# XiaoJiang-Phy/TensorCrossInterpolation.jl

Hardware: AMD Instinct MI355X
Metric: rrLU GFLOP/s at (m,n,r)=(8192,8192,256) (higher is better)
Workload: dtype f64

## Files before the change

### tensorcrossinterpolation.jl_amd/csrc/tci_rrlu.hip

```cpp
#include <hip/hip_runtime.h>
#include <math.h>
#include <stdint.h>

#include <type_traits>

#include "tci_internal.h"
#include "tci_smalllu.h"

#ifndef TCI_PASS2_U
#define TCI_PASS2_U 4
#endif
#ifndef TCI_SH_HALF
#define TCI_SH_HALF 1
#endif
#ifndef TCI_PASS_SH_U
#define TCI_PASS_SH_U 2
#endif
#ifndef TCI_SH_MFMA
#define TCI_SH_MFMA TCI_SH_HALF
#endif
#ifndef TCI_SH_NT
#define TCI_SH_NT 0
#endif
#ifndef TCI_SH_TIGHT
// ... 816 lines not shown
    const int G = kP2StageCols / cb;
    constexpr int RL = kShRL, RH = RL / 2;
    typedef float fvec __attribute__((ext_vector_type(RL)));
    typedef shT svec __attribute__((ext_vector_type(RL)));
    const int r0 = tr * kRowsPerTile + slice * kShSliceRows + RL * lane;
    const int rb = r0 < m ? r0 : 0;
    const shT* const sbase = reinterpret_cast<const shT*>(g.S) + rb;
    const int cbs = __builtin_ctz(cb);
    auto chunk_col = [&](int g0, int h) -> int {
        const int it = g0 + ((h * U) >> cbs);
        return ((q + (rev ? ntc - 1 - it : it) * nq) << cbs) + ((h * U) & (cb - 1));
    };
    auto load_chunk = [&](int g0, int h, svec (&v)[U]) {
        const int j = chunk_col(g0, h);
#pragma unroll
        for (int u = 0; u < U; ++u)
            v[u] = *reinterpret_cast<const svec*>(sbase + (int64_t)min(j + u, n - 1) * lds);
    };
    auto stage_col = [&](int g0) -> int {
        const int gn = min(G, ntc - g0);
        const int lc = threadIdx.x;
        if (lc >= gn * cb) return -1;
        const int it = g0 + (lc >> cbs);
        return ((q + (rev ? ntc - 1 - it : it) * nq) << cbs) + (lc & (cb - 1));
    };
    int rp[RL];
#pragma unroll
    for (int t = 0; t < RL; ++t) rp[t] = r0 + t < m ? sel.rowpos[r0 + t] : -1;
    const int lrow = slice * kShSliceRows + RL * lane;
    int jst = ntc > 0 ? stage_col(0) : -1;
    int cpst = (jst >= 0 && jst < n) ? colpos[jst] : -1;
    svec va[U], vb[U];
    const int nch0 = ntc > 0 ? min(G, ntc) * cb / U : 0;
    if (rep < nch0) load_chunk(0, rep, va);
    if (rep + kShReps < nch0) load_chunk(0, rep + kShReps, vb);
    if (st->done) return false;
    const int a = (int)st->p, b = (int)st->q;
    const double piv = st->pval;
    const double ypr0 = g.A[a + (int64_t)((jst >= 0 && jst < n) ? jst : 0) * lda];
    unsigned inm = 0;
#pragma unroll
    for (int t = 0; t < RL; ++t) inm |= (rp[t] > k ? 1u : 0u) << t;
    const bool active = inm != 0;
    typedef float f2v __attribute__((ext_vector_type(2)));
    f2v xf[P][RH];
    {
        double xk[RL];
#pragma unroll
        for (int hh = 0; hh < RH; ++hh) {
            const double2 c0 = *reinterpret_cast<const double2*>(g.A + rb + 2 * hh + (int64_t)b * lda);
            xk[2 * hh] = c0.x;
            xk[2 * hh + 1] = c0.y;
        }
#pragma unroll
        for (int s = 0; s < P - 1; ++s) {
            double xs[RL];
#pragma unroll
            for (int hh = 0; hh < RH; ++hh) {
                const double2 u0 = *reinterpret_cast<const double2*>(g.X + (int64_t)s * ldx + rb + 2 * hh);
                xs[2 * hh] = u0.x;
                xs[2 * hh + 1] = u0.y;
                xf[s][hh] = f2v{(float)u0.x, (float)u0.y};
            }
            const double yv = g.Y[(int64_t)s * ldy + b];
#pragma unroll
            for (int t = 0; t < RL; ++t) xk[t] = __dsub_rn(xk[t], __dmul_rn(xs[t], yv));
        }
#pragma unroll
        for (int t = 0; t < RL; ++t)
            if (g.leftorth) xk[t] = xk[t] / piv;
#pragma unroll
        for (int hh = 0; hh < RH; ++hh) xf[P - 1][hh] = f2v{(float)xk[2 * hh], (float)xk[2 * hh + 1]};
        if (rep == 0) {
#pragma unroll
            for (int t = 0; t < RL; ++t) L.xk[lrow + t] = xk[t];
            if (q == 0) {
#pragma unroll
                for (int t = 0; t < RL; ++t)
                    if (inm >> t & 1) {
                        g.X[(int64_t)(P - 1) * ldx + r0 + t] = xk[t];
                        g.Lp[r0 + t + (int64_t)k * g.ldl] = xk[t];
                    }
            }
        }
    }
    PPROF(1);
    const bool wact = __any(active);
    const float margin = 0x1p-20f;
    float tau = 0.0f;
    auto approx = [&](int h, const svec (&v)[U]) -> float {
        float cm[RL];
#pragma unroll
        for (int t = 0; t < RL; ++t) cm[t] = 0.0f;
#pragma unroll
        for (int u = 0; u < U; ++u) {
            const int lc = h * U + u;
            if (L.cpos[lc] <= k) continue;
            const fvec vf = __builtin_convertvector(v[u], fvec);
            f2v w[RH];
#pragma unroll
            for (int hh = 0; hh < RH; ++hh) w[hh] = f2v{vf[2 * hh], vf[2 * hh + 1]};
#pragma unroll
            for (int s = 0; s < P; ++s) {
                const float y = L.yf[lc * P + s];
                const f2v yy = {y, y};
#pragma unroll
                for (int hh = 0; hh < RH; ++hh) w[hh] = __builtin_elementwise_fma(-xf[s][hh], yy, w[hh]);
            }
#pragma unroll
            for (int hh = 0; hh < RH; ++hh) {
                cm[2 * hh] = fmaxf(cm[2 * hh], fabsf(w[hh].x));
                cm[2 * hh + 1] = fmaxf(cm[2 * hh + 1], fabsf(w[hh].y));
            }
        }
        float c = 0.0f;
#pragma unroll
        for (int t = 0; t < RL; ++t)
            if (inm >> t & 1) c = fmaxf(c, cm[t]);
        return c;
    };
    auto examine = [&](int g0, int e0, int e1) {
#pragma unroll 1
        for (int z = 0; z < 2; ++z) {
            const int h = z ? e1 : e0;
            if (h < 0) continue;
            int rbx = rb;
            asm volatile("" : "+v"(rbx));
            const int j0 = chunk_col(g0, h);
#pragma unroll 1
            for (int u = 0; u < U; ++u) {
                const int lc = h * U + u;
                const int cp = L.cpos[lc];
                if (cp <= k) continue;
                const int j = j0 + u;
                const double* pa = g.A + rbx + (int64_t)j * lda;
                double v[RL];
#pragma unroll
                for (int hh = 0; hh < RH; ++hh) {
                    const double2 p0 = *reinterpret_cast<const double2*>(pa + 2 * hh);
                    v[2 * hh] = p0.x;
                    v[2 * hh + 1] = p0.y;
                }
#pragma unroll 1
                for (int s = 0; s < P - 1; ++s) {
                    const double y = L.ys[lc * P + s];
#pragma unroll
                    for (int hh = 0; hh < RH; ++hh) {
                        const double2 u0 = *reinterpret_cast<const double2*>(g.X + (int64_t)s * ldx + rbx + 2 * hh);
                        v[2 * hh] = __dsub_rn(v[2 * hh], __dmul_rn(u0.x, y));
                        v[2 * hh + 1] = __dsub_rn(v[2 * hh + 1], __dmul_rn(u0.y, y));
                    }
                }
                const double yk = L.ys[lc * P + P - 1];
#pragma unroll 1
                for (int t = 0; t < RL; ++t) {
                    if (!(inm >> t & 1)) continue;
                    const double vt = __dsub_rn(v[t], __dmul_rn(L.xk[lrow + t], yk));
                    const double a2 = __dmul_rn(vt, vt);
                    if (a2 >= best.v) cand_take(best, CandR{a2, vt, cp, sel.rowpos[r0 + t], j, r0 + t});
                }
            }
        }
    };
    auto test = [&](float c) -> bool {
        const float lb = fmaxf(c - eps, 0.0f);
        const float ts = __uint_as_float(__hip_atomic_load(&L.tau, __ATOMIC_RELAXED, __HIP_MEMORY_SCOPE_WORKGROUP));
        tau = fmaxf(tau, ts);
        if (lb > tau) {
            tau = lb;
            atomicMax(&L.tau, __float_as_uint(lb));
        }
        return c + eps >= tau - tau * margin;
    };
    for (int g0 = 0; g0 < ntc; g0 += G) {
        const int gn = min(G, ntc - g0);
        const int nch = gn * cb / U;
        if (g0 > 0) {
            jst = stage_col(g0);
            cpst = (jst >= 0 && jst < n) ? colpos[jst] : -1;
            if (wact) {
                if (rep < nch) load_chunk(g0, rep, va);
                if (rep + kShReps < nch) load_chunk(g0, rep + kShReps, vb);
            }
            __syncthreads();
        }
        if (jst >= 0) {
            int lc = threadIdx.x;
            asm volatile("" : "+v"(lc));
            L.cpos[lc] = cpst;
            if (cpst > k) {
                double yk = g0 == 0 ? ypr0 : g.A[a + (int64_t)jst * lda];
#pragma unroll
                for (int s = 0; s < P - 1; ++s) {
                    const double ysv = g.Y[(int64_t)s * ldy + jst];
                    L.ys[lc * P + s] = ysv;
                    L.yf[lc * P + s] = (float)(ysv * shs);
                    yk = __dsub_rn(yk, __dmul_rn(g.X[(int64_t)s * ldx + a], ysv));
                }
                if (!g.leftorth) yk = yk / piv;
                L.ys[lc * P + P - 1] = yk;
                L.yf[lc * P + P - 1] = (float)(yk * shs);
                if (tr == 0) {
                    g.Y[(int64_t)(P - 1) * ldy + jst] = yk;
                    g.Up[k + (int64_t)jst * g.ldu] = yk;
                }
            }
        }
        if (threadIdx.x < kShSlices) L.cnt[threadIdx.x] = 2 * kShReps;
        if (g0 == 0 && threadIdx.x == 0) L.tau = 0u;
        __syncthreads();
        if (g0 == 0) PPROF(2);
        auto grab = [&]() -> int {
            int h = 0;
            if (lane == 0) h = atomicAdd(&L.cnt[slice], 1);
            return __shfl(h, 0);
        };
        int h0 = rep, h1 = rep + kShReps;
        int ex0 = -1, ex1 = -1;
        if (g0 == 0) {
            float c0 = -1.0f, c1 = -1.0f;
            const int e0 = h0, e1 = h1;
            if (wact) {
                if (h0 < nch) {
                    c0 = approx(h0, va);
                    h0 = grab();
                    if (h0 < nch) load_chunk(g0, h0, va);
                }
                if (h1 < nch) {
                    c1 = approx(h1, vb);
                    h1 = grab();
                    if (h1 < nch) load_chunk(g0, h1, vb);
                }
                float lb = fmaxf(fmaxf(c0, c1) - eps, 0.0f);
#pragma unroll
                for (int off = 32; off >= 1; off >>= 1) lb = fmaxf(lb, __shfl_xor(lb, off));
                if (lane == 0) atomicMax(&L.tau, __float_as_uint(lb));
            }
            __syncthreads();
            if (!wact) continue;
            tau = __uint_as_float(L.tau);
            if (c0 >= 0.0f && c0 + eps >= tau - tau * margin) ex0 = e0;
            if (c1 >= 0.0f && c1 + eps >= tau - tau * margin) ex1 = e1;
        } else if (!wact) {
            continue;
        }
        for (;;) {
            if (ex0 >= 0 || ex1 >= 0) examine(g0, ex0, ex1);
            ex0 = ex1 = -1;
            if (h0 >= nch) break;
            {
                const float c = approx(h0, va);
                const int e = h0;
                h0 = grab();
                if (h0 < nch) load_chunk(g0, h0, va);
                if (test(c)) ex0 = e;
            }
            if (h1 < nch) {
                const float c = approx(h1, vb);
                const int e = h1;
                h1 = grab();
                if (h1 < nch) load_chunk(g0, h1, vb);
                if (test(c)) ex1 = e;
            }
        }
    }
    return true;
}

template <int P>
__global__ __launch_bounds__(kP2Threads) void k_pass_sh(PassK g, SelArgs sel) {
    __shared__ P2Lds<P> L;
    [[maybe_unused]] unsigned long long pt[8] = {0, 0, 0, 0, 0, 0, 0, 0};
    PPROF(0);
    const double* pv = sel.pivvals;
    const int t0 = g.k - P + 1;
    const double Mf = fabs(pv[t0]);
    double sumM = 0.0;
#pragma unroll
    for (int s = 0; s < P; ++s) sumM += fabs(pv[t0 + s]);
    const double mag = Mf + 2.0 * sumM;
    const double shs = sh_scale(sh_bound(pv, t0));
    double epsd = (double)(P + 3) * 0x1p-23 * mag * shs + (double)(P + 2) * 0x1p-124;
    if (kShHalf) epsd += 0x1p-11 * (1.0 + 0x1p-10) * Mf * shs + 0x1p-25;
    const bool shok = shs > 0.0 && mag < 0x1p100 &&
                      epsd < ldexp(fabs(pv[g.k]) * shs, -(kShHalf ? TCI_SH_TIGHT : 10));
    CandR best = cand_none();
    bool go;
    if (shok)
        go = pass_sh_body<P>(g, sel, L, best, (float)(epsd * (1.0 + 0x1p-20)), shs, pt);
    else
        go = pass2_body<P, false, false>(g, sel, L, best, pt);
    if (!go) return;
    PPROF(3);
    pass_tail<kP2Threads>(best, sel, g.cand, pt, g.m, P, 0);
}

constexpr int kMfRows = 64;
constexpr int kMfBlk = kMfRows / 16;
constexpr int kMfSlices = kRowsPerTile / kMfRows;
constexpr int kMfReps = kP2Threads / 64 / kMfSlices;
static_assert(kMfBlk == 4, "a lane's 16 loaded rows are 4 blocks of 4");

constexpr int kMfMaxP = 15;
constexpr int kMfExCap = 128;
#ifndef TCI_EXB
#define TCI_EXB 4
#endif
constexpr int kExB = TCI_EXB;
static_assert(3 * kMfMaxP <= 64 && kMfMaxP < kMaxPend, "two MFMA K-steps per tile");

template <int P, bool EXT = false>
struct MfGeom {
    static constexpr bool deep = P > 10;
    static constexpr int KS = deep ? 64 : 32;
    static constexpr int KSP = KS + 8;
    static constexpr bool ymem = deep || EXT;
    static constexpr int YS = ymem ? 1 : P;
};

template <int kB>
__device__ __forceinline__ double pend_apply(double v, const double* __restrict__ xp, int64_t xst,
                                             const double* __restrict__ yp, int64_t yst, int cnt) {
    for (int s0 = 0; s0 < cnt; s0 += kB) {
        double xv[kB], yv[kB];
#pragma unroll
        for (int i = 0; i < kB; ++i)
            if (s0 + i < cnt) {
                xv[i] = xp[(int64_t)(s0 + i) * xst];
                yv[i] = yp[(int64_t)(s0 + i) * yst];
            }
#pragma unroll
        for (int i = 0; i < kB; ++i)
            if (s0 + i < cnt) v = __dsub_rn(v, __dmul_rn(xv[i], yv[i]));
    }
    return v;
}

constexpr int kPendPre = 16;
static_assert(kMaxPendR - 1 <= 2 * kPendPre, "two batches");
struct PendPre {
    double v[kPendPre];
};
template <bool COH = false>
__device__ __forceinline__ void pend_pre(PendPre& p, const double* __restrict__ xp, int64_t xst, int cnt) {
    static_assert(kPendPre <= kMaxPendR, "prefetched slots exist");
#pragma unroll
    for (int i = 0; i < kPendPre; ++i) p.v[i] = ldc<COH>(xp + (int64_t)i * xst);
#pragma unroll
    for (int i = 0; i < kPendPre; ++i)
        if (i >= cnt) p.v[i] = 0.0;
}
template <bool COH = false>
__device__ __forceinline__ double pend_chain(double v, const PendPre& p, const double* __restrict__ xp,
                                             int64_t xst, double upl, int cnt) {
#pragma unroll
    for (int i = 0; i < kPendPre; ++i)
        if (i < cnt) v = __dsub_rn(v, __dmul_rn(p.v[i], readlane_dbl(upl, i)));
    if (cnt > kPendPre) {
        double r[kMaxPendR - 1 - kPendPre];
#pragma unroll
        for (int i = 0; i < kMaxPendR - 1 - kPendPre; ++i) r[i] = ldc<COH>(xp + (int64_t)(kPendPre + i) * xst);
#pragma unroll
        for (int i = 0; i < kMaxPendR - 1 - kPendPre; ++i)
            if (kPendPre + i < cnt) v = __dsub_rn(v, __dmul_rn(r[i], readlane_dbl(upl, kPendPre + i)));
    }
    return v;
}

template <int P, bool EXT = false>
struct P2MfLds {
    using Gm = MfGeom<P, EXT>;
    double ys[kP2StageCols * Gm::YS];
    _Float16 yb[kP2StageCols * Gm::KSP];
    int cpos[kP2StageCols];
    int cnt[kMfSlices];
    unsigned tau;
    double xk[kRowsPerTile];
    union {
        _Float16 xa[kRowsPerTile * Gm::KSP];
        struct {
            unsigned ex[kP2Threads / 64 * kMfExCap];
            float exm[kP2Threads / 64 * kMfExCap];
        } e;
    } u;
};

typedef _Float16 h8v __attribute__((ext_vector_type(8)));
typedef float f4v __attribute__((ext_vector_type(4)));
typedef std::conditional<kShU8, u32x4v, h8v>::type ShVec;
constexpr int kShVecs = kShU8 ? 1 : 2;

__device__ __forceinline__ void f16_split(double v, _Float16& hi, _Float16& lo) {
    hi = (_Float16)(float)v;
    lo = (_Float16)(float)(v - (double)hi);
}

struct ShCert {
    double eps;
    double shs;
    bool ok;
};
template <bool COH = false>
__device__ __forceinline__ double sh_cert_load(const double* pv, int k, int PE) {
    const int lane = threadIdx.x & 63, ix = k - PE + lane;
    (void)lane;
    return ldc<COH>(pv + min(max(ix, 0), k));
}
__device__ __forceinline__ ShCert sh_cert(double w, int k, int PS, int PE, int nbs) {
    const int te = k - PE + 1, t0 = k - PS + 1;
    auto at = [&](int t) { return readlane_dbl(w, t - te + 1); };
    double d = 0.0;
    ShCert c{0.0, 0.0, false};
    for (int e = te;; e += nbs) {
        const bool cur = e >= t0;
        const int ke = cur ? k : e + nbs - 1;
        const int P = ke - e + 1;
        double sumM = 0.0, maxM = 0.0;
        for (int t = e; t <= ke; ++t) {
            sumM += fabs(at(t));
            maxM = fmax(maxM, fabs(at(t)));
        }
        const double B = e == 0 ? fabs(at(0)) : 2.0 * fabs(at(e - 1));
        const double s = sh_scale(B);
        const double rs = kShHalf ? (s > 0.0 ? sh_rscale(B) : 0.0) : 1.0;
        const double Mfd = fabs(at(e)) + d;
        const double mag = Mfd + 2.0 * sumM;
        double ea = 0.0;
        if (s > 0.0) {
            if constexpr (kShU8) {
                ea = d + (0.5 + 0x1p-14) * rs + 0x1p-19 * sumM + (double)P * 0x1p-24 * rs +
                     (double)(3 * P + 5) * 0x1p-23 * (mag + 384.0 * rs);
            } else {
                ea = d + 0x1p-11 * (1.0 + 0x1p-9) * Mfd + 0x1p-25 * rs + 0x1p-19 * sumM + (double)P * 0x1p-24 * rs +
                     (double)(3 * P + 4) * 0x1p-23 * mag;
            }
        }
        c.ok = s > 0.0 && mag < 0x1p100 && maxM * s <= 0x1p15 && ea * s < ldexp(fabs(at(ke)) * s, -kShTight);
        if (cur) {
            c.eps = ea * s;
            c.shs = s;
            return c;
        }
        d = c.ok ? ea : 0.0;
    }
}

constexpr int kMfStop = 0, kMfDone = 1, kMfExact = 2;
struct EpochIn {
    int a, b;
    double piv;
    const int32_t* lrow;
    const int16_t* lcol;
    const double* lpiv;
    int k0;
    __device__ __forceinline__ double pivot(const double* pv, int t) const { return t > k0 ? lpiv[t - k0 - 1] : pv[t]; }
};
template <int P, bool EXT = false, bool RF = false, bool COH = false>
__device__ __forceinline__ int pass_mf_body(const PassK& g, const SelArgs& sel, P2MfLds<P, EXT>& L,
                                            CandR& best, unsigned long long (&pt)[8], const int Pr = P,
                                            const EpochIn* ep = nullptr) {
    static_assert(P >= 1 && P <= kMfMaxP, "at most two MFMA K-steps per tile");
    using Gm = MfGeom<P, EXT>;
    const int PE = EXT ? g.pe : Pr;
    const int off = PE - Pr;
    constexpr int KS = Gm::KS, KSP = Gm::KSP, KSt = KS / 32;
    RrluState* st = sel.st;
    const int32_t* colpos = sel.colpos;
    const int32_t* rowpos = sel.rowpos;
    const double* pv = sel.pivvals;
    const int m = g.m, n = g.n, k = g.k, cb = g.cb, rev = g.rev, leftorth = g.leftorth;
    const int64_t lda = g.lda, ldx = g.ldx, ldy = g.ldy, lds = g.lds;
    const int t0 = k - Pr + 1;
    double certw;
    int st_done, a, bq;
    double piv;
    if constexpr (COH) {
        certw = ep->pivot(pv, min(max(k - PE + (int)(threadIdx.x & 63), 0), k));
        st_done = 0;
        a = ep->a;
        bq = ep->b;
        piv = ep->piv;
    } else {
        certw = sh_cert_load<COH>(pv, k, PE);
        st_done = ldc<true>(&st->done);
        a = (int)ldc<true>(&st->p);
        bq = (int)ldc<true>(&st->q);
        piv = ldc<true>(&st->pval);
    }
#if TCI_PASS_PROF
    if (threadIdx.x == 0) asm volatile("" ::"s"(a), "s"(bq));
#endif
    PPROFX(0);
    int tx = (int)threadIdx.x, bx = (int)blockIdx.x, gx = (int)gridDim.x;
    if constexpr (COH) asm volatile("" : "+v"(tx), "+s"(bx), "+s"(gx));
    const int lane = tx & 63, wave = tx >> 6;
    const int slice = wave % kMfSlices, rep = wave / kMfSlices;
    const int tiles_r = (m + kRowsPerTile - 1) / kRowsPerTile;
    const int tiles_c = (n + cb - 1) / cb;
    const int nq = gx / tiles_r;
    const int wid = xcd_spread(bx, gx);
    const int tr = wid % tiles_r;
    const int q = (rev && !COH) ? nq - 1 - wid / tiles_r : wid / tiles_r;
    const int ntc = q < tiles_c ? (tiles_c - 1 - q) / nq + 1 : 0;
    const int G = kP2StageCols / cb;
    const int cbs = __builtin_ctz(cb);
    const int tb = tr * kRowsPerTile;
    const int sb = tb + slice * kMfRows;
    const int gq = lane >> 4, lcol = lane & 15;
    const int rl = sb + 16 * gq;
    const bool rload = rl < lds;
    const shT* const sbase = reinterpret_cast<const shT*>(g.S) + (rload ? rl : 0);
    auto col_of = [&](int g0, int lc) -> int {
        const int it = g0 + (lc >> cbs);
        return ((q + (rev ? ntc - 1 - it : it) * nq) << cbs) + (lc & (cb - 1));
    };
    [[maybe_unused]] auto lcol_of = [&](int g0, int lc) -> int {
        const int it = g0 + (lc >> cbs);
        return ((rev ? ntc - 1 - it : it) << cbs) + (lc & (cb - 1));
    };
    auto rowpos_of = [&](int r) -> int {
        if constexpr (COH)
            return ep->lrow[r - tb];
        else
            return rowpos[r];
    };
    auto load_chunk = [&](int g0, int gcols, int h, ShVec (&v)[kShVecs]) {
        const int lc = h * 16 + lcol;
        const int j = lc < gcols ? col_of(g0, lc) : n;
        const ShVec* p = reinterpret_cast<const ShVec*>(sbase + (int64_t)(j < n ? j : n - 1) * lds);
#pragma unroll
        for (int i = 0; i < kShVecs; ++i) v[i] = p[i];
    };
    const bool stager = tx < kP2StageCols;
    auto stage_col = [&](int g0) -> int {
        const int gn = min(G, ntc - g0);
        const int lc = tx;
        if (!stager || lc >= gn * cb) return -1;
        return col_of(g0, lc);
    };
    int rpa[kMfBlk];
#pragma unroll
    for (int b = 0; b < kMfBlk; ++b) rpa[b] = rowpos_of(min(sb + 16 * (lcol >> 2) + 4 * b + (lcol & 3), m - 1));
    [[maybe_unused]] int rpt[RF ? 16 : 1];
    if constexpr (RF) {
#pragma unroll
        for (int i = 0; i < 16; ++i) rpt[i] = rowpos_of(min(rl + i, m - 1));
    }
    [[maybe_unused]] const int shb = (int)(unsigned)min((int64_t)lds * n * (int64_t)sizeof(shT), (int64_t)0xFFFFFFF0);
    [[maybe_unused]] const auto rsS0 = buf_rsrc(g.S, shb);
    [[maybe_unused]] const auto rsS1 = buf_rsrc(reinterpret_cast<const char*>(g.S) + 16, shb - 16);
    int jst = ntc > 0 ? stage_col(0) : -1;
    int cpl;
    if constexpr (COH)
        cpl = ep->lcol[jst >= 0 ? lcol_of(0, tx) : 0];
    else
        cpl = colpos[min(max(jst, 0), n - 1)];
    const int prow = tx - kP2StageCols;
    const int rrow = tb + (prow >= 0 ? prow : 0);
    const int rpl = rowpos_of(min(rrow, m - 1));
    ShVec va[kShVecs], vb[kShVecs];
    const int gc0 = ntc > 0 ? min(G, ntc) * cb : 0;
    const int nch0 = (gc0 + 15) / 16;
    load_chunk(0, gc0, max(min(rep, nch0 - 1), 0), va);
    load_chunk(0, gc0, max(min(rep + kMfReps, nch0 - 1), 0), vb);
    [[maybe_unused]] PendPre pre;
    if constexpr (EXT) {
        pend_pre<COH>(pre, stager ? g.Y + (jst >= 0 && jst < n ? jst : 0) : g.X + (rrow < m ? rrow : 0),
                 stager ? ldy : ldx, PE - 1);
    }
    PPROFX(1);
    const int ac = min(max(a, 0), m - 1), bc = min(max(bq, 0), n - 1);
    const int jj = jst >= 0 && jst < n ? jst : 0;
    [[maybe_unused]] double upl = 0.0;
    if constexpr (EXT) {
        upl = ldc<COH>((stager ? g.X + ac : g.Y + bc) + (int64_t)min(lane, kMaxPendR - 1) * (stager ? ldx : ldy));
    }
    double a0 = 0.0;
    if (!stager)
        a0 = g.A[(rrow < m ? rrow : 0) + (int64_t)bc * lda];
    else if constexpr (EXT)
        a0 = g.A[ac + (int64_t)jj * lda];
    const ShCert cert = sh_cert(certw, k, Pr, PE, g.nbs > 0 ? g.nbs : Pr);
#if TCI_PASS_PROF
    if (threadIdx.x == 0) asm volatile("" ::"v"(cert.eps));
#endif
    PPROFX(2);
#ifdef TCI_EPOCH_DEBUG
    {
        const double c0 = readlane_dbl(certw, 0), c1 = readlane_dbl(certw, 1), c2 = readlane_dbl(certw, 2),
                     c3 = readlane_dbl(certw, 3), c4 = readlane_dbl(certw, 4);
        if (tx == 0 && bx == 0 && k < 12)
            printf("[%s k=%d Pr=%d PE=%d nbs=%d] cert ok=%d eps=%g shs=%g pv lanes %.17g %.17g %.17g %.17g %.17g\n",
                   COH ? "epoch" : "pass", k, Pr, PE, g.nbs, (int)cert.ok, cert.eps, cert.shs, c0, c1, c2, c3, c4);
    }
#endif
    if (!cert.ok) return kMfExact;
    const float eps = (float)(cert.eps * (1.0 + 0x1p-20));
    const double shs = cert.shs;
    [[maybe_unused]] const float rscale =
        RF ? (float)(sh_scale(sh_bound(pv, k + 1)) / shs) : 1.0f;
    if (st_done) return kMfStop;
    PPROF(6);
    if (!stager) {
        const int rr = rrow < m ? rrow : 0;
        double xs[P];
        if constexpr (!EXT) {
#pragma unroll
            for (int s = 0; s < P - 1; ++s)
                if (s < Pr - 1) xs[s] = ldc<COH>(g.X + (int64_t)(off + s) * ldx + rr);
        }
        double xk = a0;
        if constexpr (EXT) {
#pragma unroll
            for (int s = 0; s < P - 1; ++s)
                if (s < Pr - 1) xs[s] = ldc<COH>(g.X + (int64_t)(off + s) * ldx + rr);
            xk = pend_chain<COH>(xk, pre, g.X + rr, ldx, upl, PE - 1);
        } else {
#pragma unroll
            for (int s = 0; s < P - 1; ++s)
                if (s < Pr - 1) xk = __dsub_rn(xk, __dmul_rn(xs[s], ldc<COH>(g.Y + (int64_t)s * ldy + bq)));
        }
        if (leftorth) xk = xk / piv;
        L.xk[prow] = xk;
        const int rpos = rrow < m ? rpl : -1;
        if (q == 0 && rpos > k) {
            stc<COH>(g.X + (int64_t)(PE - 1) * ldx + rrow, xk);
            g.Lp[rrow + (int64_t)k * g.ldl] = xk;
        }
#pragma unroll
        for (int s = 0; s < P; ++s)
            if (s == Pr - 1) xs[s] = xk;
        const int dd = rpos > k ? Pr : (rpos >= t0 ? rpos - t0 : -1);
        double own = 0.0;
        if (!leftorth) {
            if constexpr (COH)
                own = rpos >= t0 && rpos <= k ? ep->pivot(pv, rpos) : 0.0;
            else
                own = rpos >= t0 && rpos <= k ? pv[rpos] : 0.0;
        } else {
            own = 1.0;
        }
        _Float16 sl[KS];
#pragma unroll
        for (int s = 0; s < P; ++s) {
            double x = s < dd ? xs[s] : (s == dd ? own : 0.0);
            if (s >= Pr) x = 0.0;
            x = -(leftorth ? x : x * shs);
            f16_split(x, sl[3 * s], sl[3 * s + 2]);
            sl[3 * s + 1] = sl[3 * s];
        }
#pragma unroll
        for (int z = 3 * P; z < KS; ++z) sl[z] = (_Float16)0.0f;
        if constexpr (kShU8) sl[3 * P] = (_Float16)1.0f;
#pragma unroll
        for (int z = 0; z < KS / 8; ++z) {
            h8v w;
#pragma unroll
            for (int e = 0; e < 8; ++e) w[e] = sl[8 * z + e];
            *reinterpret_cast<h8v*>(&L.u.xa[prow * KSP + 8 * z]) = w;
        }
    }
    [[maybe_unused]] double yk0 = 0.0;
    PPROFX(3);
    if constexpr (EXT) {
        if (stager) yk0 = pend_chain<COH>(a0, pre, g.Y + jj, ldy, upl, PE - 1);
    }
    PPROF(1);
    bool act = false;
#pragma unroll
    for (int b = 0; b < kMfBlk; ++b) act |= sb + 16 * (lcol >> 2) + 4 * b + (lcol & 3) < m && rpa[b] > k;
    [[maybe_unused]] unsigned tmask = 0;
    if constexpr (RF) {
#pragma unroll
        for (int i = 0; i < 16; ++i) tmask |= (rl + i < m && rpt[i] > k ? 1u : 0u) << i;
    }
    int cpst = (jst >= 0 && jst < n) ? cpl : -1;
    const bool wact = RF || __any(act);
    const float margin = 0x1p-20f;
    float tau = 0.0f;
    h8v af[kMfBlk][KSt];
    int g0r = 0;
    auto approx = [&](int h, int gcols, const ShVec (&v)[kShVecs], float (&mbs)[kMfBlk]) -> float {
        const int lc = h * 16 + lcol;
        const int cp = lc < gcols ? L.cpos[lc] : -1;
        h8v bf[KSt];
#pragma unroll
        for (int u = 0; u < KSt; ++u)
            bf[u] = *reinterpret_cast<const h8v*>(&L.yb[(lc < gcols ? lc : 0) * KSP + 32 * u + 8 * gq]);
        float c = 0.0f;
        [[maybe_unused]] h8v wout[2];
        [[maybe_unused]] u32x4v wq;
#pragma unroll
        for (int b = 0; b < kMfBlk; ++b) {
            f4v acc;
            if constexpr (kShU8) {
                const uint32_t d = __builtin_bit_cast(u32x4v, v[0])[b];
                acc = f4v{(float)(d & 0xFFu), (float)((d >> 8) & 0xFFu), (float)((d >> 16) & 0xFFu), (float)(d >> 24)};
                if (!rload) acc = f4v{128.0f, 128.0f, 128.0f, 128.0f};
            } else {
                const h8v hv = __builtin_bit_cast(h8v, v[(b >> 1) % kShVecs]);
                const int o = 4 * (b & 1);
                acc = f4v{(float)hv[o], (float)hv[o + 1], (float)hv[o + 2], (float)hv[o + 3]};
                if (!rload) acc = f4v{0.0f, 0.0f, 0.0f, 0.0f};
            }
#pragma unroll
            for (int u = 0; u < KSt; ++u) acc = __builtin_amdgcn_mfma_f32_16x16x32_f16(af[b][u], bf[u], acc, 0, 0, 0);
            mbs[b] = __builtin_fmaxf(__builtin_fmaxf(fabsf(acc[0]), fabsf(acc[1])),
                                     __builtin_fmaxf(fabsf(acc[2]), fabsf(acc[3])));
            c = __builtin_fmaxf(c, mbs[b]);
            if constexpr (RF) {
                if constexpr (kShU8) {
                    uint32_t q = 0;
#pragma unroll
                    for (int t = 0; t < 4; ++t)
                        q |= ((tmask >> (4 * b + t)) & 1u ? sh_u8(acc[t] * rscale) : kShU8Zero) << (8 * t);
                    wq[b] = q;
                } else {
                    const int o = 4 * (b & 1);
#pragma unroll
                    for (int t = 0; t < 4; ++t)
                        wout[b >> 1][o + t] = (tmask >> (4 * b + t)) & 1u ? (_Float16)(acc[t] * rscale) : (_Float16)0.0f;
                }
            }
        }
        if constexpr (RF) {
            const int j = lc < gcols ? col_of(g0r, lc) : n;
            const unsigned off =
                rload && j < n && cp > k ? (unsigned)(((int64_t)j * lds + rl) * (int64_t)sizeof(shT)) : 0xFFFFFFF0u;
            if constexpr (kShU8) {
                __builtin_amdgcn_raw_buffer_store_b128(wq, rsS0, (int)off, 0, 0);
            } else {
                __builtin_amdgcn_raw_buffer_store_b128(__builtin_bit_cast(u32x4v, wout[0]), rsS0, (int)off, 0, 0);
                __builtin_amdgcn_raw_buffer_store_b128(__builtin_bit_cast(u32x4v, wout[1]), rsS1, (int)off, 0, 0);
            }
        }
        if (cp <= k) {
#pragma unroll
            for (int b = 0; b < kMfBlk; ++b) mbs[b] = -1.0f;
            c = -1.0f;
        }
        return c;
    };
    unsigned* const exl = L.u.e.ex + wave * kMfExCap;
    float* const exm = L.u.e.exm + wave * kMfExCap;
    int nex = 0;
    auto flush = [&](int g0, auto fast) {
        const float thr = tau - tau * margin;
        for (int e = lane; e < 4 * nex; e += 64) {
            const unsigned key = exl[e >> 2];
            if (exm[e >> 2] + eps < thr) continue;
            const int lc = (int)(key & 1023u), rq = (int)(key >> 10);
            const int r = sb + 4 * rq + (e & 3);
            if (r >= m) continue;
            const int j = col_of(g0, lc);
            double v = g.A[r + (int64_t)j * lda];
            const int rp = rowpos_of(r);
            asm volatile("" : "+v"(v));
            if (rp <= k) continue;
            if constexpr (decltype(fast)::value) {
                if constexpr (Gm::ymem) {
                    for (int s0 = 0; s0 < PE - 1; s0 += kExB) {
                        double xv[kExB], yv[kExB];
#pragma unroll
                        for (int i = 0; i < kExB; ++i)
                            if (s0 + i < PE - 1) {
                                xv[i] = ldc<COH>(g.X + (int64_t)(s0 + i) * ldx + r);
                                yv[i] = ldc<COH>(g.Y + (int64_t)(s0 + i) * ldy + j);
                            }
#pragma unroll
                        for (int i = 0; i < kExB; ++i)
                            if (s0 + i < PE - 1) v = __dsub_rn(v, __dmul_rn(xv[i], yv[i]));
                    }
                } else {
                    double xv[P];
#pragma unroll
                    for (int s = 0; s < P - 1; ++s)
                        if (s < Pr - 1) xv[s] = ldc<COH>(g.X + (int64_t)s * ldx + r);
#pragma unroll
                    for (int s = 0; s < P - 1; ++s)
                        if (s < Pr - 1) v = __dsub_rn(v, __dmul_rn(xv[s], L.ys[lc * P + s]));
                }
            } else {
#pragma unroll 1
                for (int s = 0; s < PE - 1; ++s)
                    v = __dsub_rn(v, __dmul_rn(ldc<COH>(g.X + (int64_t)s * ldx + r),
                                               Gm::ymem ? ldc<COH>(g.Y + (int64_t)s * ldy + j) : L.ys[lc * P + s]));
            }
            v = __dsub_rn(v, __dmul_rn(L.xk[r - tb], L.ys[lc * Gm::YS + Gm::YS - 1]));
            const double a2 = __dmul_rn(v, v);
            if (a2 >= best.v) cand_take(best, CandR{a2, v, L.cpos[lc], rp, j, r});
#if TCI_PASS_PROF
            atomicAdd(&g_exam_lds, 1u);
#endif
        }
        nex = 0;
    };
    auto append = [&](int g0, int h, const float (&mbs)[kMfBlk], float bound) {
        const unsigned lc = (unsigned)(h * 16 + lcol);
#pragma unroll
        for (int b = 0; b < kMfBlk; ++b) {
            const bool f = mbs[b] >= 0.0f && mbs[b] + eps >= bound;
            const uint64_t bal = __ballot(f);
            if (bal == 0) continue;
            const int cnt = __popcll(bal);
            if (nex + cnt > kMfExCap) flush(g0, std::false_type{});
            if (f) {
                const int at = nex + (int)__builtin_amdgcn_mbcnt_hi((unsigned)(bal >> 32),
                                                                    __builtin_amdgcn_mbcnt_lo((unsigned)bal, 0u));
                exl[at] = lc | (unsigned)(4 * gq + b) << 10;
                exm[at] = mbs[b];
            }
            nex += cnt;
        }
    };
    auto test = [&](float c) {
        if (c < 0.0f) return;
        const float lb = fmaxf(c - eps, 0.0f);
        const float ts = __uint_as_float(__hip_atomic_load(&L.tau, __ATOMIC_RELAXED, __HIP_MEMORY_SCOPE_WORKGROUP));
        tau = fmaxf(tau, ts);
        if (lb > tau) {
            tau = lb;
            atomicMax(&L.tau, __float_as_uint(lb));
        }
    };
    for (int g0 = 0; g0 < ntc; g0 += G) {
        const int gn = min(G, ntc - g0);
        const int gcols = gn * cb;
        const int nch = (gcols + 15) / 16;
        g0r = g0;
        if (g0 > 0) {
            jst = stage_col(g0);
            if constexpr (COH)
                cpst = jst >= 0 ? ep->lcol[lcol_of(g0, tx)] : -1;
            else
                cpst = (jst >= 0 && jst < n) ? colpos[jst] : -1;
            load_chunk(g0, gcols, min(rep, nch - 1), va);
            load_chunk(g0, gcols, min(rep + kMfReps, nch - 1), vb);
            __syncthreads();
        }
        [[maybe_unused]] double ykg = yk0;
        if constexpr (EXT) {
            if (g0 > 0 && stager) {
                const int jj = jst >= 0 && jst < n ? jst : 0;
                PendPre pg;
                pend_pre<COH>(pg, g.Y + jj, ldy, PE - 1);
                ykg = pend_chain<COH>(g.A[a + (int64_t)jj * lda], pg, g.Y + jj, ldy, upl, PE - 1);
            }
        }
        if (jst >= 0) {
            int lc = tx;
            asm volatile("" : "+v"(lc));
            L.cpos[lc] = cpst;
            if (cpst > k) {
                double ysv[P];
#pragma unroll
                for (int s = 0; s < P - 1; ++s)
                    if (s < Pr - 1) ysv[s] = ldc<COH>(g.Y + (int64_t)(off + s) * ldy + jst);
                double yk;
                if constexpr (EXT) {
                    yk = ykg;
                } else {
                    yk = g.A[a + (int64_t)jst * lda];
#pragma unroll
                    for (int s = 0; s < P - 1; ++s)
                        if (s < Pr - 1) yk = __dsub_rn(yk, __dmul_rn(ldc<COH>(g.X + (int64_t)s * ldx + a), ysv[s]));
                }
                if (!leftorth) yk = yk / piv;
#pragma unroll
                for (int s = 0; s < P; ++s)
                    if (s == Pr - 1) ysv[s] = yk;
                if (tr == 0) {
                    stc<COH>(g.Y + (int64_t)(PE - 1) * ldy + jst, yk);
                    g.Up[k + (int64_t)jst * g.ldu] = yk;
                }
                _Float16 sl[KS];
                L.ys[lc * Gm::YS + Gm::YS - 1] = yk;
#pragma unroll
                for (int s = 0; s < P; ++s) {
                    if (s < Pr) {
                        if constexpr (!Gm::ymem) L.ys[lc * P + s] = ysv[s];
                        f16_split(leftorth ? ysv[s] * shs : ysv[s], sl[3 * s], sl[3 * s + 1]);
                    } else {
                        sl[3 * s] = sl[3 * s + 1] = (_Float16)0.0f;
                    }
                    sl[3 * s + 2] = sl[3 * s];
                }
#pragma unroll
                for (int z = 3 * P; z < KS; ++z) sl[z] = (_Float16)0.0f;
                if constexpr (kShU8) sl[3 * P] = (_Float16)-128.0f;
#pragma unroll
                for (int z = 0; z < KS / 8; ++z) {
                    h8v w;
#pragma unroll
                    for (int e = 0; e < 8; ++e) w[e] = sl[8 * z + e];
                    *reinterpret_cast<h8v*>(&L.yb[lc * KSP + 8 * z]) = w;
                }
            }
        }
        if (g0 == 0) PPROF(7);
        if (tx < kMfSlices) L.cnt[tx] = 2 * kMfReps;
        if (g0 == 0 && tx == 0) L.tau = 0u;
        __syncthreads();
        if (g0 == 0) {
#pragma unroll
            for (int b = 0; b < kMfBlk; ++b) {
                const int pr = slice * kMfRows + 16 * (lcol >> 2) + 4 * b + (lcol & 3);
#pragma unroll
                for (int u = 0; u < KSt; ++u)
                    af[b][u] = *reinterpret_cast<const h8v*>(&L.u.xa[pr * KSP + 32 * u + 8 * gq]);
            }
            PPROF(2);
        }
        auto grab = [&]() -> int {
            int h = 0;
            if (lane == 0) h = atomicAdd(&L.cnt[slice], 1);
            return __builtin_amdgcn_readfirstlane(h);
        };
        int h0 = rep, h1 = rep + kMfReps;
        float mb0[kMfBlk], mb1[kMfBlk];
        if (g0 == 0) {
            float c0 = -1.0f, c1 = -1.0f;
            const int e0 = h0, e1 = h1;
#pragma unroll
            for (int b = 0; b < kMfBlk; ++b) mb0[b] = mb1[b] = -1.0f;
            if (wact) c0 = approx(h0, gcols, va, mb0);
            h0 = grab();
            load_chunk(g0, gcols, min(h0, nch - 1), va);
            if (wact && (RF || EXT || h1 < nch)) c1 = approx(h1, gcols, vb, mb1);
            h1 = grab();
            load_chunk(g0, gcols, min(h1, nch - 1), vb);
            if (wact) {
                float lb = fmaxf(fmaxf(c0, c1) - eps, 0.0f);
#pragma unroll
                for (int off = 32; off >= 1; off >>= 1) lb = fmaxf(lb, __shfl_xor(lb, off));
                if (lane == 0) atomicMax(&L.tau, __float_as_uint(lb));
            }
            __syncthreads();
            if (!wact) continue;
            tau = __uint_as_float(L.tau);
            const float bound = tau - tau * margin;
            if (e0 < nch) append(g0, e0, mb0, bound);
            if (e1 < nch) append(g0, e1, mb1, bound);
        } else if (!wact) {
            continue;
        }
        while (h0 < nch) {
            {
                const float c = approx(h0, gcols, va, mb0);
                const int e = h0;
                h0 = grab();
                load_chunk(g0, gcols, min(h0, nch - 1), va);
                test(c);
                append(g0, e, mb0, tau - tau * margin);
            }
            {
                const int e = h1;
                float c = -1.0f;
                if (RF || EXT || e < nch) c = approx(e, gcols, vb, mb1);
                h1 = grab();
                load_chunk(g0, gcols, min(h1, nch - 1), vb);
                if (RF || EXT || e < nch) {
                    test(c);
                    append(g0, e, mb1, tau - tau * margin);
                }
            }
        }
        tau = fmaxf(tau, __uint_as_float(__hip_atomic_load(&L.tau, __ATOMIC_RELAXED, __HIP_MEMORY_SCOPE_WORKGROUP)));
        flush(g0, std::true_type{});
    }
    return kMfDone;
}

constexpr int kXHalf = 256;
#ifndef TCI_XSTAGE
#define TCI_XSTAGE 128
#endif
#ifndef TCI_PX_EXP
#define TCI_PX_EXP 0
#endif
constexpr int kXStage = TCI_XSTAGE;
#ifndef TCI_PX_DRAIN
#define TCI_PX_DRAIN 1
#endif
#ifndef TCI_XU
#define TCI_XU 4
#endif
constexpr int kXU = TCI_XU;
static_assert(kXU == 4 || kXU == 8, "chunks of 4 or 8 columns (cb is a multiple of 8)");
constexpr int kXSlices = kXHalf / 128;
constexpr int kXReps = kP2Threads / 64 / kXSlices;
template <int NT>
struct PxGeom {
    static constexpr int Half = NT == 1024 ? 256 : 128;
    static constexpr int Tile = 2 * Half;
    static constexpr int Slices = Half / 128;
    static constexpr int Reps = NT / 64 / Slices;
};
template <int NT>
struct alignas(16) PxLdsT {
    alignas(16) double xs[kMaxPendR * PxGeom<NT>::Half];
    alignas(16) double ys[kMaxPendR * kXStage];
    double xa[kMaxPendR];
    double yb[kMaxPendR];
    int cpos[kXStage];
    int cnt[PxGeom<NT>::Slices];
};
using PxLds = PxLdsT<kP2Threads>;

template <int MODE, bool COH = false, int NT = kP2Threads>
__device__ __forceinline__ bool passx_body(const PassK& g, const SelArgs& sel, PxLdsT<NT>& L, CandR& best,
                                           unsigned long long (&pt)[8]) {
    constexpr int kXHalf = PxGeom<NT>::Half, kXSlices = PxGeom<NT>::Slices, kXReps = PxGeom<NT>::Reps;
    constexpr int kRowsPerTile = PxGeom<NT>::Tile, kP2Threads = NT;
    RrluState* st = sel.st;
    const int32_t* rowpos = sel.rowpos;
    const int32_t* colpos = sel.colpos;
    double* __restrict__ A = g.A;
    const int64_t lda = g.lda, ldx = g.ldx, ldy = g.ldy;
    const int m = g.m, n = g.n, k = g.k, cb = g.cb, rev = g.rev, leftorth = g.leftorth;
    const int P = g.pe;
    const int lane = threadIdx.x & 63, wave = __builtin_amdgcn_readfirstlane(threadIdx.x >> 6);
    const int slice = wave % kXSlices, rep = wave / kXSlices;
    const int tiles_r = (m + kRowsPerTile - 1) / kRowsPerTile;
    const int tiles_c = (n + cb - 1) / cb;
    const int nq = gridDim.x / tiles_r;
    const int wid = xcd_spread(blockIdx.x, gridDim.x);
    const int tr = wid % tiles_r;
    const int q = rev ? nq - 1 - wid / tiles_r : wid / tiles_r;
    const int ntc = q < tiles_c ? (tiles_c - 1 - q) / nq + 1 : 0;
    const int G = kXStage / cb;
    const int cbs = __builtin_ctz(cb);
    auto col_of = [&](int g0, int lc) -> int {
        const int it = g0 + (lc >> cbs);
        return ((q + (rev ? ntc - 1 - it : it) * nq) << cbs) + (lc & (cb - 1));
    };
    if (st->done) return false;
    const int a = (int)st->p, b = (int)st->q;
    const double piv = st->pval;
    if (threadIdx.x < P - 1) {
        L.xa[threadIdx.x] = g.X[(int64_t)threadIdx.x * ldx + a];
        L.yb[threadIdx.x] = g.Y[(int64_t)threadIdx.x * ldy + b];
    }
    [[maybe_unused]] const double shs = MODE ? sh_scale(sh_bound(sel.pivvals, k + 1)) : 1.0;
    PPROF(1);
    for (int half = 0; half < kRowsPerTile / kXHalf; ++half) {
        const int hb = tr * kRowsPerTile + half * kXHalf;
        if (hb >= m) break;
        __syncthreads();
        {
            constexpr int kPer = kMaxPendR * kXHalf / kP2Threads;
            double v[kPer];
#pragma unroll
            for (int u = 0; u < kPer; ++u) {
                const int e = threadIdx.x + u * kP2Threads, s = e / kXHalf, rr = e - s * kXHalf;
                v[u] = g.X[(int64_t)s * ldx + min(hb + rr, m - 1)];
                if (!(s < P - 1 && hb + rr < m)) v[u] = 0.0;
            }
#pragma unroll
            for (int u = 0; u < kPer; ++u) {
                const int e = threadIdx.x + u * kP2Threads;
                if (e < (P - 1) * kXHalf) L.xs[e] = v[u];
            }
        }
        __syncthreads();
        if (threadIdx.x < kXHalf) {
            const int rr = threadIdx.x, r = hb + rr;
            double xk = 0.0;
            if (r < m) {
                xk = A[r + (int64_t)b * lda];
                for (int s = 0; s < P - 1; ++s) xk = __dsub_rn(xk, __dmul_rn(L.xs[s * kXHalf + rr], L.yb[s]));
                if (leftorth) xk = xk / piv;
                if (q == 0 && rowpos[r] > k) {
                    stc<COH>(g.X + (int64_t)(P - 1) * ldx + r, xk);
                    g.Lp[r + (int64_t)k * g.ldl] = xk;
                }
            }
            L.xs[(P - 1) * kXHalf + rr] = xk;
        }
        const int lr = slice * 128 + 2 * lane;
        const int r0 = hb + lr;
        const bool rowok = r0 < m, pair = r0 + 1 < m;
        const int rp0 = rowok ? rowpos[r0] : -1, rp1 = pair ? rowpos[r0 + 1] : -1;
        const bool in0 = rp0 > k, in1 = rp1 > k;
        const bool wact = MODE != 0 || __any(in0 || in1);
        const uint32_t roff = rowok ? r0 : 0;
        for (int g0 = 0; g0 < ntc; g0 += G) {
            const int gcols = min(G, ntc - g0) * cb;
            const int nch = gcols / kXU;
            if (g0 > 0) __syncthreads();
            {
                constexpr int kPer = kMaxPendR * kXStage / kP2Threads;
                const int lc = threadIdx.x & (kXStage - 1), s0 = threadIdx.x / kXStage;
                const int j = lc < gcols ? col_of(g0, lc) : 0;
                double v[kPer];
#pragma unroll
                for (int u = 0; u < kPer; ++u) {
                    const int s = s0 + u * (kP2Threads / kXStage);
                    v[u] = g.Y[(int64_t)s * ldy + j];
                    if (!(s < P - 1 && lc < gcols)) v[u] = 0.0;
                }
#pragma unroll
                for (int u = 0; u < kPer; ++u) {
                    const int s = s0 + u * (kP2Threads / kXStage);
                    if (s < P - 1) L.ys[s * kXStage + lc] = v[u];
                }
            }
            const int lcs = threadIdx.x, js = lcs < gcols ? col_of(g0, lcs) : 0;
            const int cps = (lcs < gcols && js < n) ? colpos[js] : -1;
            const double ypr = (lcs < gcols && cps > k) ? A[a + (int64_t)js * lda] : 0.0;
            __syncthreads();
            if (lcs < gcols) {
                L.cpos[lcs] = cps;
                if (cps > k) {
                    double yk = ypr;
                    for (int s = 0; s < P - 1; ++s) yk = __dsub_rn(yk, __dmul_rn(L.xa[s], L.ys[s * kXStage + lcs]));
                    if (!leftorth) yk = yk / piv;
                    L.ys[(P - 1) * kXStage + lcs] = yk;
                    if (tr == 0 && half == 0) {
                        stc<COH>(g.Y + (int64_t)(P - 1) * ldy + js, yk);
                        g.Up[k + (int64_t)js * g.ldu] = yk;
                    }
                }
            }
            if (threadIdx.x < kXSlices) L.cnt[threadIdx.x] = 2 * kXReps;
            __syncthreads();
            if (g0 == 0 && half == 0) PPROF(2);
            if (!wact) continue;
            auto load_chunk = [&](int h, double2 (&v)[kXU]) {
                const int j0 = col_of(g0, h * kXU);
#pragma unroll
                for (int u = 0; u < kXU; ++u) {
                    const double* colp = A + (int64_t)min(j0 + u, n - 1) * lda;
                    const double2* pa = reinterpret_cast<const double2*>(colp + roff);
                    if constexpr (MODE == 1 && TCI_FLUSH_NTL) {
                        typedef double dv2 __attribute__((ext_vector_type(2)));
                        const dv2 w = __builtin_nontemporal_load(reinterpret_cast<const dv2*>(pa));
                        v[u] = double2{w.x, w.y};
                    } else {
                        v[u] = *pa;
                    }
                }
            };
            auto process = [&](int h, double2 (&v)[kXU]) {
                int cp[kXU];
                bool any = false;
#pragma unroll
                for (int u = 0; u < kXU; ++u) {
                    cp[u] = __builtin_amdgcn_readfirstlane(L.cpos[h * kXU + u]);
                    any |= cp[u] > k;
                }
                if (!any) return;
                const int j0 = col_of(g0, h * kXU);
#pragma unroll 2
                for (int s = 0; s < P; ++s) {
#if TCI_PX_EXP & 1
                    const dv2 x = dv2{1.0 + s, 0.5 * s};
#else
                    const dv2 x = *reinterpret_cast<const dv2*>(
                        __builtin_assume_aligned(&L.xs[s * kXHalf + lr], 16));
#endif
                    double y[kXU];
#pragma unroll
                    for (int u = 0; u < kXU; u += 2) {
#if TCI_PX_EXP & 2
                        const dv2 yy = dv2{0.25 * s + u, 0.125 * s};
#else
                        const dv2 yy = *reinterpret_cast<const dv2*>(
                            __builtin_assume_aligned(&L.ys[s * kXStage + h * kXU + u], 16));
#endif
                        y[u] = yy.x;
                        y[u + 1] = yy.y;
                    }
#pragma unroll
                    for (int u = 0; u < kXU; ++u) {
                        v[u].x = __dsub_rn(v[u].x, __dmul_rn(x.x, y[u]));
                        v[u].y = __dsub_rn(v[u].y, __dmul_rn(x.y, y[u]));
                    }
                }
                double mx0 = 0.0, mx1 = 0.0;
#pragma unroll
                for (int u = 0; u < kXU; ++u) {
                    if (cp[u] <= k) continue;
                    const int j = j0 + u;
                    if constexpr (MODE == 1) {
                        if (in0 || in1) {
                            double2* pa = reinterpret_cast<double2*>(A + (int64_t)j * lda + roff);
                            if (!in1) {
                                pa->x = v[u].x;
                            } else if (!in0) {
                                pa->y = v[u].y;
                            } else {
                                typedef double dv2 __attribute__((ext_vector_type(2)));
                                dv2 w = {v[u].x, v[u].y};
                                __builtin_nontemporal_store(w, reinterpret_cast<dv2*>(pa));
                            }
                        }
                    }
                    if constexpr (MODE != 0 && kShU8) {
                        if (rowok) {
                            uint8_t* ps = reinterpret_cast<uint8_t*>(g.S) + (int64_t)j * g.lds + roff;
                            const uint32_t c0 = in0 ? sh_u8((float)(v[u].x * shs)) : kShU8Zero;
                            if (pair)
                                *reinterpret_cast<uint16_t*>(ps) =
                                    (uint16_t)(c0 | (in1 ? sh_u8((float)(v[u].y * shs)) : kShU8Zero) << 8);
                            else
                                ps[0] = (uint8_t)c0;
                        }
                    } else if constexpr (MODE != 0 && kShHalf) {
                        if (rowok) {
                            _Float16* ps = reinterpret_cast<_Float16*>(g.S) + (int64_t)j * g.lds + roff;
                            const _Float16 h0 = in0 ? (_Float16)(float)(v[u].x * shs) : (_Float16)0.0f;
                            if (pair) {
                                typedef _Float16 h2v __attribute__((ext_vector_type(2)));
                                *reinterpret_cast<h2v*>(ps) = h2v{h0, in1 ? (_Float16)(float)(v[u].y * shs) : (_Float16)0.0f};
                            } else {
                                ps[0] = h0;
                            }
                        }
                    }
                    mx0 = fmax(mx0, fabs(v[u].x));
                    mx1 = fmax(mx1, fabs(v[u].y));
                }
                const double mx = fmax(in0 ? mx0 : 0.0, in1 ? mx1 : 0.0);
                if (__dmul_rn(mx, mx) >= best.v) {
#pragma unroll
                    for (int u = 0; u < kXU; ++u) {
                        if (cp[u] <= k) continue;
                        const int j = j0 + u;
                        const double a0 = __dmul_rn(v[u].x, v[u].x), a1 = __dmul_rn(v[u].y, v[u].y);
                        if ((in0 && a0 >= best.v) || (in1 && a1 >= best.v)) {
                            if (in0) cand_take(best, CandR{a0, v[u].x, cp[u], rp0, j, r0});
                            if (in1) cand_take(best, CandR{a1, v[u].y, cp[u], rp1, j, r0 + 1});
                        }
                    }
                }
            };
            auto grab = [&]() -> int {
                int h = 0;
                if (lane == 0) h = atomicAdd(&L.cnt[slice], 1);
                return __builtin_amdgcn_readfirstlane(h);
            };
            double2 va[kXU], vb[kXU];
            int h0 = rep, h1 = rep + kXReps;
#if TCI_PX_DRAIN
            if (h0 < nch) load_chunk(h0, va);
            while (h0 < nch) {
                __builtin_amdgcn_s_waitcnt(0x0f70);
                if (h1 < nch) load_chunk(h1, vb);
                process(h0, va);
                if (h1 >= nch) break;
                h0 = grab();
                __builtin_amdgcn_s_waitcnt(0x0f70);
                if (h0 < nch) load_chunk(h0, va);
                process(h1, vb);
                h1 = grab();
            }
#else
            if (h0 < nch) load_chunk(h0, va);
            if (h1 < nch) load_chunk(h1, vb);
            while (h0 < nch) {
                process(h0, va);
                h0 = grab();
                if (h0 < nch) load_chunk(h0, va);
                if (h1 >= nch) break;
                process(h1, vb);
                h1 = grab();
                if (h1 < nch) load_chunk(h1, vb);
            }
// ... 998 lines not shown
```

Before: 2690.

## Generalize MFMA screening pass to a configurable depth of in-flight chunk buffers

After: 2882 (median of 6 runs). 1.07x the previous value.

```diff
diff --git a/tensorcrossinterpolation.jl_amd/csrc/tci_rrlu.hip b/tensorcrossinterpolation.jl_amd/csrc/tci_rrlu.hip
--- a/tensorcrossinterpolation.jl_amd/csrc/tci_rrlu.hip
+++ b/tensorcrossinterpolation.jl_amd/csrc/tci_rrlu.hip
@@ -1142,6 +1142,11 @@
 static_assert(kMfBlk == 4, "a lane's 16 loaded rows are 4 blocks of 4");
 
 constexpr int kMfMaxP = 15;
+#ifndef TCI_MF_INFLIGHT
+#define TCI_MF_INFLIGHT 2
+#endif
+constexpr int kMfInflight = TCI_MF_INFLIGHT;
+static_assert(kMfInflight >= 2 && kMfInflight <= 8, "the seed consumes two buffers; each costs 4-8 VGPRs");
 constexpr int kMfExCap = 128;
 #ifndef TCI_EXB
 #define TCI_EXB 4
@@ -1156,6 +1161,10 @@
     static constexpr int KSP = KS + 8;
     static constexpr bool ymem = deep || EXT;
     static constexpr int YS = ymem ? 1 : P;
+};
+template <int P, bool EXT, bool RF>
+struct MfDepth {
+    static constexpr int D = P > 10 ? 2 : kMfInflight;
 };
 
 template <int kB>
@@ -1398,11 +1407,12 @@
     const int prow = tx - kP2StageCols;
     const int rrow = tb + (prow >= 0 ? prow : 0);
     const int rpl = rowpos_of(min(rrow, m - 1));
-    ShVec va[kShVecs], vb[kShVecs];
+    constexpr int D = MfDepth<P, EXT, RF>::D;
+    ShVec vbuf[D][kShVecs];
     const int gc0 = ntc > 0 ? min(G, ntc) * cb : 0;
     const int nch0 = (gc0 + 15) / 16;
-    load_chunk(0, gc0, max(min(rep, nch0 - 1), 0), va);
-    load_chunk(0, gc0, max(min(rep + kMfReps, nch0 - 1), 0), vb);
+    load_chunk(0, gc0, max(min(rep, nch0 - 1), 0), vbuf[0]);
+    load_chunk(0, gc0, max(min(rep + kMfReps, nch0 - 1), 0), vbuf[1]);
     [[maybe_unused]] PendPre pre;
     if constexpr (EXT) {
         pend_pre<COH>(pre, stager ? g.Y + (jst >= 0 && jst < n ? jst : 0) : g.X + (rrow < m ? rrow : 0),
@@ -1506,6 +1516,8 @@
         if (stager) yk0 = pend_chain<COH>(a0, pre, g.Y + jj, ldy, upl, PE - 1);
     }
     PPROF(1);
+#pragma unroll
+    for (int i = 2; i < D; ++i) load_chunk(0, gc0, max(min(rep + i * kMfReps, nch0 - 1), 0), vbuf[i]);
     bool act = false;
 #pragma unroll
     for (int b = 0; b < kMfBlk; ++b) act |= sb + 16 * (lcol >> 2) + 4 * b + (lcol & 3) < m && rpa[b] > k;
@@ -1536,7 +1548,6 @@
             if constexpr (kShU8) {
                 const uint32_t d = __builtin_bit_cast(u32x4v, v[0])[b];
                 acc = f4v{(float)(d & 0xFFu), (float)((d >> 8) & 0xFFu), (float)((d >> 16) & 0xFFu), (float)(d >> 24)};
-                if (!rload) acc = f4v{128.0f, 128.0f, 128.0f, 128.0f};
             } else {
                 const h8v hv = __builtin_bit_cast(h8v, v[(b >> 1) % kShVecs]);
                 const int o = 4 * (b & 1);
@@ -1545,8 +1556,11 @@
             }
 #pragma unroll
             for (int u = 0; u < KSt; ++u) acc = __builtin_amdgcn_mfma_f32_16x16x32_f16(af[b][u], bf[u], acc, 0, 0, 0);
-            mbs[b] = __builtin_fmaxf(__builtin_fmaxf(fabsf(acc[0]), fabsf(acc[1])),
-                                     __builtin_fmaxf(fabsf(acc[2]), fabsf(acc[3])));
+            mbs[b] = __builtin_fmaxf(__builtin_fmaxf(__builtin_fmaxf(fabsf(acc[0]), fabsf(acc[1])), fabsf(acc[2])),
+                                     fabsf(acc[3]));
+            if constexpr (kShU8) {
+                if (!rload) mbs[b] = 0.0f;
+            }
             c = __builtin_fmaxf(c, mbs[b]);
             if constexpr (RF) {
                 if constexpr (kShU8) {
@@ -1637,6 +1651,9 @@
     };
     auto append = [&](int g0, int h, const float (&mbs)[kMfBlk], float bound) {
         const unsigned lc = (unsigned)(h * 16 + lcol);
+        const float mx = __builtin_fmaxf(__builtin_fmaxf(__builtin_fmaxf(mbs[0], mbs[1]), mbs[2]), mbs[3]);
+        static_assert(kMfBlk == 4, "mx covers every block");
+        if (__ballot(mx >= 0.0f && mx + eps >= bound) == 0) return;
 #pragma unroll
         for (int b = 0; b < kMfBlk; ++b) {
             const bool f = mbs[b] >= 0.0f && mbs[b] + eps >= bound;
@@ -1674,8 +1691,8 @@
                 cpst = jst >= 0 ? ep->lcol[lcol_of(g0, tx)] : -1;
             else
                 cpst = (jst >= 0 && jst < n) ? colpos[jst] : -1;
-            load_chunk(g0, gcols, min(rep, nch - 1), va);
-            load_chunk(g0, gcols, min(rep + kMfReps, nch - 1), vb);
+#pragma unroll
+            for (int i = 0; i < D; ++i) load_chunk(g0, gcols, min(rep + i * kMfReps, nch - 1), vbuf[i]);
             __syncthreads();
         }
         [[maybe_unused]] double ykg = yk0;
@@ -1738,7 +1755,7 @@
             }
         }
         if (g0 == 0) PPROF(7);
-        if (tx < kMfSlices) L.cnt[tx] = 2 * kMfReps;
+        if (tx < kMfSlices) L.cnt[tx] = D * kMfReps;
         if (g0 == 0 && tx == 0) L.tau = 0u;
         __syncthreads();
         if (g0 == 0) {
@@ -1756,19 +1773,34 @@
             if (lane == 0) h = atomicAdd(&L.cnt[slice], 1);
             return __builtin_amdgcn_readfirstlane(h);
         };
-        int h0 = rep, h1 = rep + kMfReps;
-        float mb0[kMfBlk], mb1[kMfBlk];
+        int h[D];
+#pragma unroll
+        for (int i = 0; i < D; ++i) h[i] = rep + i * kMfReps;
+        auto turn = [&](int i, bool first) {
+            const int e = h[i];
+            float mbs[kMfBlk];
+            float c = -1.0f;
+            const bool on = first || RF || EXT || e < nch;
+            if (on) c = approx(e, gcols, vbuf[i], mbs);
+            h[i] = grab();
+            load_chunk(g0, gcols, min(h[i], nch - 1), vbuf[i]);
+            if (on) {
+                test(c);
+                append(g0, e, mbs, tau - tau * margin);
+            }
+        };
         if (g0 == 0) {
             float c0 = -1.0f, c1 = -1.0f;
-            const int e0 = h0, e1 = h1;
+            float mb0[kMfBlk], mb1[kMfBlk];
+            const int e0 = h[0], e1 = h[1];
 #pragma unroll
             for (int b = 0; b < kMfBlk; ++b) mb0[b] = mb1[b] = -1.0f;
-            if (wact) c0 = approx(h0, gcols, va, mb0);
-            h0 = grab();
-            load_chunk(g0, gcols, min(h0, nch - 1), va);
-            if (wact && (RF || EXT || h1 < nch)) c1 = approx(h1, gcols, vb, mb1);
-            h1 = grab();
-            load_chunk(g0, gcols, min(h1, nch - 1), vb);
+            if (wact) c0 = approx(e0, gcols, vbuf[0], mb0);
+            h[0] = grab();
+            load_chunk(g0, gcols, min(h[0], nch - 1), vbuf[0]);
+            if (wact && (RF || EXT || e1 < nch)) c1 = approx(e1, gcols, vbuf[1], mb1);
+            h[1] = grab();
+            load_chunk(g0, gcols, min(h[1], nch - 1), vbuf[1]);
             if (wact) {
                 float lb = fmaxf(fmaxf(c0, c1) - eps, 0.0f);
 #pragma unroll
@@ -1781,29 +1813,14 @@
             const float bound = tau - tau * margin;
             if (e0 < nch) append(g0, e0, mb0, bound);
             if (e1 < nch) append(g0, e1, mb1, bound);
+#pragma unroll
+            for (int i = 2; i < D; ++i) turn(i, false);
         } else if (!wact) {
             continue;
         }
-        while (h0 < nch) {
-            {
-                const float c = approx(h0, gcols, va, mb0);
-                const int e = h0;
-                h0 = grab();
-                load_chunk(g0, gcols, min(h0, nch - 1), va);
-                test(c);
-                append(g0, e, mb0, tau - tau * margin);
-            }
-            {
-                const int e = h1;
-                float c = -1.0f;
-                if (RF || EXT || e < nch) c = approx(e, gcols, vb, mb1);
-                h1 = grab();
-                load_chunk(g0, gcols, min(h1, nch - 1), vb);
-                if (RF || EXT || e < nch) {
-                    test(c);
-                    append(g0, e, mb1, tau - tau * margin);
-                }
-            }
+        while (h[0] < nch) {
+#pragma unroll
+            for (int i = 0; i < D; ++i) turn(i, i == 0);
         }
         tau = fmaxf(tau, __uint_as_float(__hip_atomic_load(&L.tau, __ATOMIC_RELAXED, __HIP_MEMORY_SCOPE_WORKGROUP)));
         flush(g0, std::true_type{});
```
